# Liz490/multimodal_alzheimer

Measured on AMD Instinct MI355X. Metric: volumes/sec fwd+bwd, 3D-ResNet-10 @128^3 bf16, 1/2/4/8 MI355X; % HBM roofline, higher is better.
Workload: dtype bf16; 1 GPU; BASELINE config 2: Anat_CNN ResNet-10 MRI-only, 1x128^3, batch 8/GPU, weighted CE, Adam, fwd+bwd+step; global_batch=8, parallelism=dp1, step_launch=hip graph replay

## Files before the change

multimodal_alzheimer_amd/csrc/pwgrad.hip:

```cpp
#include "common.h"
#include "patchconv.h"

namespace {

constexpr int PW_KC = 32;
constexpr int PW_TY = 8;
constexpr int PW_XW = 32;
constexpr int PW_YR = PW_TY + 2;
constexpr int PW_XSLOTS = 4;
constexpr int PW_YROW = 128;
constexpr int PW_YST = 2 * PW_XW * PW_YROW;
constexpr int PW_YSLOTS = 4;
constexpr int PW_NTHR = 512;
constexpr uint32_t PW_OOB = 0x80000000u;
template <int MODE>
struct PWC {
  static constexpr bool LAT = MODE == 1, W16 = MODE == 2, W40 = MODE == 3;
  static constexpr int XR = LAT ? 40 : W16 ? 18 : W40 ? 50 : PW_XW + 2;
  static constexpr int SPP = W40 ? 5 : 4;
  static constexpr int YRI = W16 ? 18 : PW_YR;
  static constexpr int XROWS = YRI * XR;
  static constexpr int XDMA = (XROWS + 15) / 16;
  static constexpr int XSLOT = XDMA * 1024;
  static constexpr int Y_OFF = PW_XSLOTS * XSLOT;
  static constexpr int LDS = Y_OFF + PW_YSLOTS * PW_YST;
  static constexpr int NXMAX = (XDMA + 7) / 8;
};

struct PWG {
  int nb, Cs, Nd, D, H, K;
  int zr;
  int ng;
};

__device__ __forceinline__ int pw_wsz128(int r) { return 2 * ((r >> 1) & 1) + 4 * ((r >> 3) & 1); }

template <int MODE>
__global__ __launch_bounds__(PW_NTHR) void pwgrad_kernel(PWG g, const u16* __restrict__ x,
                                                         const u16* __restrict__ dy,
                                                         float* __restrict__ ws) {
  using C = PWC<MODE>;
  constexpr bool LAT = C::LAT, W16 = C::W16, W40 = C::W40;
  constexpr int XR = C::XR, SPP = C::SPP;
  extern __shared__ __attribute__((aligned(16))) char smem[];
  const int tid = threadIdx.x, lane = tid & 63;
  const int wave = __builtin_amdgcn_readfirstlane(tid >> 6);
  const int nci = g.Cs / PW_KC, nco = g.Nd / 64;
  const int nwg = gridDim.x, bid = blockIdx.x;
  const int xcd = bid & 7, qq = nwg >> 3, rr = nwg & 7;
  const int tile = (xcd < rr ? xcd * (qq + 1) : rr * (qq + 1) + (xcd - rr) * qq) + (bid >> 3);
  const int cot = tile % nco, t2 = tile / nco;
  const int cit = t2 % nci, split = t2 / nci;
  const int nyt = LAT ? 2 / g.ng : W16 ? 1 : g.H / PW_TY, nzr = (LAT ? 8 : g.D) / g.zr;
  const int zi = split % nzr, yt = (split / nzr) % nyt, n = split / (nzr * nyt);
  const int rz = LAT ? yt : 0;
  const int co0 = cot * 64, ci0 = cit * PW_KC, y0 = LAT || W16 ? 0 : yt * PW_TY, z0 = zi * g.zr;
  constexpr int VW = LAT || W16 ? 16 : W40 ? 40 : PW_XW;

  const int64_t vox = LAT ? (int64_t)16 * 16 * 16 : (int64_t)g.D * g.H * VW;
  const __amdgpu_buffer_rsrc_t rsx = __builtin_amdgcn_make_buffer_rsrc(
      (void*)(x + n * vox * g.Cs), 0, (int)__builtin_amdgcn_readfirstlane((int)(vox * g.Cs * 2)),
      0x00020000);
  const __amdgpu_buffer_rsrc_t rsy = __builtin_amdgcn_make_buffer_rsrc(
      (void*)(dy + n * vox * g.Nd), 0, (int)__builtin_amdgcn_readfirstlane((int)(vox * g.Nd * 2)),
      0x00020000);
  const uint32_t smem_l = lds_addr_of(smem);

  const int nx = wave + 8 * (C::NXMAX - 1) < C::XDMA ? C::NXMAX : C::NXMAX - 1;
  auto xoff = [&](int h) -> uint32_t {
    const int q = wave + 8 * h, row = 16 * q + (lane >> 2);
    if constexpr (LAT) {
      const int yv = row / XR - 1, ps = row % XR, sg = ps / 10, xv = ps % 10 - 1;
      const bool ok = row < C::XROWS && (unsigned)yv < 8u && (unsigned)xv < 8u;
      const int vy = (sg >> 1) + 2 * yv, vx = (sg & 1) + 2 * xv;
      return ok ? (uint32_t)(((vy * 16 + vx) * g.Cs + ci0 + (lane & 3) * 8) * 2) : PW_OOB;
    } else if constexpr (W16) {
      const int yv = row / XR - 1, xv = row % XR - 1;
      const bool ok = row < C::XROWS && (unsigned)yv < (unsigned)g.H && (unsigned)xv < 16u;
      return ok ? (uint32_t)(((yv * 16 + xv) * g.Cs + ci0 + (lane & 3) * 8) * 2) : PW_OOB;
    } else if constexpr (W40) {
      const int yv = y0 - 1 + row / XR, ps = row % XR, xv = 8 * (ps / 10) + ps % 10 - 1;
      const bool ok = row < C::XROWS && (unsigned)yv < (unsigned)g.H && (unsigned)xv < 40u;
      return ok ? (uint32_t)(((yv * 40 + xv) * g.Cs + ci0 + (lane & 3) * 8) * 2) : PW_OOB;
    } else {
      const int yv = y0 - 1 + row / XR, xv = row % XR - 1;
      const bool ok = row < C::XROWS && (unsigned)yv < (unsigned)g.H &&
                      (unsigned)xv < (unsigned)PW_XW;
      return ok ? (uint32_t)(((yv * PW_XW + xv) * g.Cs + ci0 + (lane & 3) * 8) * 2) : PW_OOB;
    }
  };
  const uint32_t xplane = LAT ? (uint32_t)(16 * 16 * g.Cs * 2) : (uint32_t)(g.H * VW * g.Cs * 2);
  const int gstride = g.zr + 2;
  auto issue_x = [&](int e, int rz) {
    const uint32_t slot = smem_l + (uint32_t)(((unsigned)e % PW_XSLOTS) * C::XSLOT);
    if (LAT && e >= gstride) {
      e -= gstride;
      rz += 1;
    }
    const int zp = z0 - 1 + e;
    const bool zin = !LAT || (unsigned)zp < 8u;
    const uint32_t pz = LAT ? (uint32_t)(rz + 2 * zp) * xplane : (uint32_t)zp * xplane;
#pragma unroll
    for (int h = 0; h < C::NXMAX; ++h)
      if (h < nx)
        buf_lds16_asm(zin ? xoff(h) + pz : PW_OOB, rsx, slot + (uint32_t)((wave + 8 * h) * 1024));
  };
  const int yr = wave * 8 + (lane >> 3);
  const int yvox = LAT ? ((((yr >> 3) & 3) >> 1) + 2 * (yr >> 5)) * 16 + (((yr >> 3) & 3) & 1) +
                             2 * (yr & 7)
                       : yr;
  const uint32_t ylane = (uint32_t)(((W40 ? (lane >> 3) : yvox) * g.Nd + co0 +
                                     ((lane & 7) ^ pw_wsz128(yr)) * 8) * 2);
  auto issue_y = [&](int o, int m, int sl, int rz) {
    uint32_t base;
    if constexpr (W40) {
      const int j = 4 * (2 * m + (wave >> 2)) + (wave & 3);
      base = (uint32_t)((((z0 + o) * g.H + y0 + j / 5) * 40 + 8 * (j % 5)) * g.Nd * 2);
    } else {
      base = LAT ? (uint32_t)(((rz + 2 * (z0 + o)) * 16 + 4 * m) * 16) * (uint32_t)g.Nd * 2
             : W16 ? (uint32_t)(((z0 + o) * g.H + 4 * m) * 16) * (uint32_t)g.Nd * 2
                   : (uint32_t)(((z0 + o) * g.H + y0 + 2 * m) * PW_XW) * (uint32_t)g.Nd * 2;
    }
    buf_lds16_asm(base + ylane, rsy, smem_l + (uint32_t)(C::Y_OFF + sl * PW_YST + wave * 1024));
  };

  const int cf = wave & 1, tg = wave >> 1;
  const int t0 = tg * 7, nt = tg == 3 ? 6 : 7;
  const int lk = lane >> 4, q4 = (lane & 15) >> 2, p4 = lane & 3;
  const int rsel = 8 * lk + q4;
  uint32_t ya_lo[4], ya_hi[4];
#pragma unroll
  for (int i = 0; i < 4; ++i) {
    const int col = i * 16 + 4 * p4;
    ya_lo[i] = (uint32_t)(rsel * PW_YROW + (((col >> 3) ^ pw_wsz128(rsel)) << 4) + (col & 7) * 2);
    ya_hi[i] = (uint32_t)((rsel + 4) * PW_YROW + (((col >> 3) ^ pw_wsz128(rsel + 4)) << 4) +
                          (col & 7) * 2);
  }
  const uint32_t xb = (uint32_t)((LAT ? 10 * lk + q4 : W16 ? 18 * (lk >> 1) + 8 * (lk & 1) + q4
                                  : W40 ? q4 : rsel) *
                                     64 + cf * 32 + 8 * p4);
  uint32_t xk[W40 ? 5 : 1];
#pragma unroll
  for (int kt = 0; kt < (W40 ? 5 : 1); ++kt) {
    const int j = 4 * kt + lk;
    xk[kt] = W40 ? (uint32_t)(((j / 5) * XR + (j % 5) * 10) * 64) : 0u;
  }
  f32x4 acc[4][7];
#pragma unroll
  for (int i = 0; i < 4; ++i)
#pragma unroll
    for (int k = 0; k < 7; ++k) acc[i][k] = f32x4{0.f, 0.f, 0.f, 0.f};

  auto tr8 = [](const char* p) {
    return __builtin_amdgcn_ds_read_tr16_b64_v4bf16((LDS_AS bf16x4*)p);
  };
  auto prologue = [&](int rz) {
    issue_x(0, rz);
    issue_x(1, rz);
    issue_x(2, rz);
    issue_y(0, 0, 0, rz);
    issue_y(0, 1, 1, rz);
  };
  prologue(rz);
  const int ng = LAT ? g.ng : 1;
  const int nstage = ng * g.zr * SPP;

  struct PFr { bf16x8 a[4], b[7]; };
  auto run = [&](auto tgc) {
    constexpr int TG = decltype(tgc)::value;
    constexpr int NT = TG == 3 ? 6 : 7;
    const char* xbase[3];
    auto y_on = [](int t, int yl) constexpr {
      return !LAT || ((unsigned)(yl + (t / 3) % 3 - 1) < 8u);
    };
    auto kread = [&](const char* yimg, auto qc, auto ylc, PFr& f) {
      constexpr int Q = decltype(qc)::value, YL = decltype(ylc)::value;
#pragma unroll
      for (int i = 0; i < 4; ++i)
        f.a[i] = __builtin_shufflevector(tr8(yimg + Q * PW_XW * PW_YROW + ya_lo[i]),
                                         tr8(yimg + Q * PW_XW * PW_YROW + ya_hi[i]), 0, 1, 2, 3,
                                         4, 5, 6, 7);
      auto one = [&](auto kc) {
        constexpr int K = decltype(kc)::value;
        if constexpr (K < NT && y_on(TG * 7 + K, YL)) {
          constexpr int t = TG * 7 + K;
          constexpr int kz = t / 9, ky = (t / 3) % 3, kx = t % 3;
          const char* img;
          if constexpr (W40) {
            constexpr int r0 = ((YL / 5) * 4 + ky) * XR + kx;
            img = xbase[kz] + xk[YL % 5] + r0 * 64;
          } else {
            constexpr int r0 = ((W16 ? 2 : 1) * YL + ky) * XR + kx;
            img = xbase[kz] + r0 * 64;
          }
          f.b[K] = __builtin_shufflevector(tr8(img), tr8(img + 4 * 64), 0, 1, 2, 3, 4, 5, 6, 7);
        }
      };
      one(std::integral_constant<int, 0>{});
      one(std::integral_constant<int, 1>{});
      one(std::integral_constant<int, 2>{});
      one(std::integral_constant<int, 3>{});
      one(std::integral_constant<int, 4>{});
      one(std::integral_constant<int, 5>{});
      one(std::integral_constant<int, 6>{});
    };
    auto kmma = [&](const PFr& f, auto ylc) {
      constexpr int YL = decltype(ylc)::value;
      auto one = [&](auto kc) {
        constexpr int K = decltype(kc)::value;
        if constexpr (K < NT && y_on(TG * 7 + K, YL)) {
#pragma unroll
          for (int i = 0; i < 4; ++i)
            acc[i][K] = __builtin_amdgcn_mfma_f32_16x16x32_bf16(f.a[i], f.b[K], acc[i][K], 0, 0,
                                                                0);
        }
      };
      one(std::integral_constant<int, 0>{});
      one(std::integral_constant<int, 1>{});
      one(std::integral_constant<int, 2>{});
      one(std::integral_constant<int, 3>{});
      one(std::integral_constant<int, 4>{});
      one(std::integral_constant<int, 5>{});
      one(std::integral_constant<int, 6>{});
    };
#pragma unroll 1
    for (int o = 0; o < ng * g.zr; ++o) {
      const bool second = o >= g.zr;
      const int v = o + (second ? 2 : 0);
      if (LAT && o == g.zr) {
        raw_barrier();
        issue_x(v + 1, rz);
        issue_x(v + 2, rz);
      }
#pragma unroll
      for (int j = 0; j < 3; ++j) {
        uint32_t b = (uint32_t)(((unsigned)(v + j) % PW_XSLOTS) * C::XSLOT) + xb;
        asm volatile("v_mov_b32 %0, %1" : "=v"(b) : "v"(b));
        xbase[j] = smem + b;
      }
      const bool xnext = v + 3 < ng * gstride;
      auto stage = [&](auto mc) {
        constexpr int M = decltype(mc)::value;
        const int s = o * SPP + M;
        if (s + 1 >= nstage || (LAT && M == 0 && o == g.zr)) {
          wait_vm_lgkm0<0>();
        } else if ((M == 1 || M == 2) && xnext) {
          if (nx == 4) wait_vm_lgkm0<5>();
          else if (nx == 3) wait_vm_lgkm0<4>();
          else wait_vm_lgkm0<3>();
        } else {
          wait_vm_lgkm0<1>();
        }
        raw_barrier();
        if (s + 2 < nstage) {
          const int p2 = (int)((unsigned)(s + 2) / SPP), g2 = p2 >= g.zr ? 1 : 0;
          issue_y(p2 - g2 * g.zr, (int)((unsigned)(s + 2) % SPP), (int)((unsigned)(s + 2) % PW_YSLOTS), rz + g2);
        }
        if (M == 0 && xnext) issue_x(v + 3, rz);
        int yoff = C::Y_OFF + (int)((unsigned)s % PW_YSLOTS) * PW_YST;
        asm volatile("" : "+s"(yoff));
        const char* yimg = smem + yoff;
        PFr f0, f1;
        kread(yimg, std::integral_constant<int, 0>{}, std::integral_constant<int, 2 * M>{}, f0);
        kread(yimg, std::integral_constant<int, 1>{}, std::integral_constant<int, 2 * M + 1>{},
              f1);
        kmma(f0, std::integral_constant<int, 2 * M>{});
        kmma(f1, std::integral_constant<int, 2 * M + 1>{});
      };
      stage(std::integral_constant<int, 0>{});
      stage(std::integral_constant<int, 1>{});
      stage(std::integral_constant<int, 2>{});
      stage(std::integral_constant<int, 3>{});
      if constexpr (SPP == 5) stage(std::integral_constant<int, 4>{});
    }
  };
  switch (tg) {
    case 0: run(std::integral_constant<int, 0>{}); break;
    case 1: run(std::integral_constant<int, 1>{}); break;
    case 2: run(std::integral_constant<int, 2>{}); break;
    default: run(std::integral_constant<int, 3>{}); break;
  }

  float* out = ws + (int64_t)split * g.Nd * g.K;
  const int lr = lane & 15;
#pragma unroll
  for (int k = 0; k < 7; ++k) {
    if (k < nt) {
      const int kcol = (t0 + k) * g.Cs + ci0 + cf * 16 + lr;
#pragma unroll
      for (int i = 0; i < 4; ++i)
#pragma unroll
        for (int r = 0; r < 4; ++r)
          out[(int64_t)(co0 + i * 16 + lk * 4 + r) * g.K + kcol] = acc[i][k][r];
    }
  }
}

bool pw_on() {
  static const bool v = [] {
    const char* e = getenv("MMAD_PWGRAD");
    return e == nullptr || atoi(e) != 0;
  }();
  return v;
}
bool lat_on() {
  static const bool v = [] {
    const char* e = getenv("MMAD_PWGRAD_LAT");
    return e == nullptr || atoi(e) != 0;
  }();
  return v;
}

bool w16_on() {
  static const bool v = [] {
    const char* e = getenv("MMAD_PWGRAD_W16");
    return e == nullptr || atoi(e) != 0;
  }();
  return v;
}
bool w16_geo(const mmad_patch::Geo& q) {
  return q.KD == 3 && q.KH == 3 && q.KW == 3 && q.dd == 1 && q.dh == 1 && q.dw == 1 &&
         q.pd == 1 && q.ph == 1 && q.pw == 1 && q.Ds == q.Dd && q.Hs == q.Hd && q.Ws == q.Wd &&
         q.Wd == 16 && q.Hd == 16 && q.Dd >= 4;
}
bool w40_on() {
  static const bool v = [] {
    const char* e = getenv("MMAD_PWGRAD_W40");
    return e == nullptr || atoi(e) != 0;
  }();
  return v;
}
bool w40_geo(const mmad_patch::Geo& q) {
  return q.KD == 3 && q.KH == 3 && q.KW == 3 && q.dd == 1 && q.dh == 1 && q.dw == 1 &&
         q.pd == 1 && q.ph == 1 && q.pw == 1 && q.Ds == q.Dd && q.Hs == q.Hd && q.Ws == q.Wd &&
         q.Wd == 40 && q.Hd % PW_TY == 0 && q.Dd >= 4;
}
bool lat_geo(const mmad_patch::Geo& q) {
  return q.KD == 3 && q.KH == 3 && q.KW == 3 && q.dd == 2 && q.dh == 2 && q.dw == 2 &&
         q.pd == 2 && q.ph == 2 && q.pw == 2 && q.Ds == 16 && q.Hs == 16 && q.Ws == 16 &&
         q.Dd == 16 && q.Hd == 16 && q.Wd == 16;
}

int lat_ng(const mmad_patch::Geo& q) {
  static const int force1 = [] {
    const char* e = getenv("MMAD_PWGRAD_LAT_NG");
    return e != nullptr && atoi(e) == 1;
  }();
  if (!lat_geo(q) || force1) return 1;
  return (int64_t)q.nb * (q.Cs / PW_KC) * (q.Nd / 64) >= 256 ? 2 : 1;
}

int pw_zr(const mmad_patch::Geo& q) {
  if (lat_geo(q)) {
    const int64_t base = (int64_t)q.nb * (2 / lat_ng(q)) * (q.Cs / PW_KC) * (q.Nd / 64);
    int zr = 8;
    while (zr > 2 && base * (8 / zr) < 256) zr /= 2;
    return zr;
  }
  const int64_t base =
      (int64_t)q.nb * (w16_geo(q) ? 1 : q.Hd / PW_TY) * (q.Cs / PW_KC) * (q.Nd / 64);
  int zr = q.Dd;
  while (zr > 4 && zr % 2 == 0 && base * (q.Dd / zr) < 256) zr /= 2;
  return zr;
}

}

namespace mmad_pwgrad {

bool ok(const mmad_patch::Geo& q) {
  if (!pw_on()) return false;
  if (q.Cs % PW_KC || q.Nd % 64 || q.Kpad != 27 * q.Cs) return false;
  if (lat_geo(q)) return lat_on() && (int64_t)4096 * std::max(q.Cs, q.Nd) * 2 < (int64_t(1) << 30);
  if (w16_geo(q)) {
    if (!w16_on() || (int64_t)q.Dd * 256 * std::max(q.Cs, q.Nd) * 2 >= (int64_t(1) << 30))
      return false;
    const int zr = pw_zr(q);
    return q.Dd % zr == 0 && zr >= 2;
  }
  if (w40_geo(q)) {
    if (!w40_on() || (int64_t)q.Dd * q.Hd * 40 * std::max(q.Cs, q.Nd) * 2 >= (int64_t(1) << 30))
      return false;
    const int zr = pw_zr(q);
    return q.Dd % zr == 0 && zr >= 2;
  }
  if (q.KD != 3 || q.KH != 3 || q.KW != 3 || q.dd != 1 || q.dh != 1 || q.dw != 1) return false;
  if (q.pd != 1 || q.ph != 1 || q.pw != 1) return false;
  if (q.Ds != q.Dd || q.Hs != q.Hd || q.Ws != q.Wd || q.Wd != PW_XW) return false;
  if (q.Hd % PW_TY || q.Dd < 4) return false;
  if ((int64_t)q.Dd * q.Hd * PW_XW * std::max(q.Cs, q.Nd) * 2 >= (int64_t(1) << 30)) return false;
  const int zr = pw_zr(q);
  return q.Dd % zr == 0 && zr >= 2;
}

int64_t splits(const mmad_patch::Geo& q) {
  if (lat_geo(q)) return (int64_t)q.nb * (2 / lat_ng(q)) * (8 / pw_zr(q));
  if (w16_geo(q)) return (int64_t)q.nb * (q.Dd / pw_zr(q));
  return (int64_t)q.nb * (q.Hd / PW_TY) * (q.Dd / pw_zr(q));
}

int64_t workspace(const mmad_patch::Geo& q) {
  return mmad_pwgrad::splits(q) * q.Nd * 27 * q.Cs * 4;
}

int wgrad(const mmad_patch::Geo& q, const void* x, const void* dy, float* ws, int* nsplit,
          void* stream) {
  if (!mmad_pwgrad::ok(q)) return MMAD_EUNSUPPORTED;
  static const bool attr =
      hipFuncSetAttribute((const void*)pwgrad_kernel<0>,
                          hipFuncAttributeMaxDynamicSharedMemorySize, PWC<0>::LDS) == hipSuccess &&
      hipFuncSetAttribute((const void*)pwgrad_kernel<1>,
                          hipFuncAttributeMaxDynamicSharedMemorySize, PWC<1>::LDS) == hipSuccess &&
      hipFuncSetAttribute((const void*)pwgrad_kernel<2>,
                          hipFuncAttributeMaxDynamicSharedMemorySize, PWC<2>::LDS) == hipSuccess &&
      hipFuncSetAttribute((const void*)pwgrad_kernel<3>,
                          hipFuncAttributeMaxDynamicSharedMemorySize, PWC<3>::LDS) == hipSuccess;
  if (!attr) return MMAD_EUNSUPPORTED;
  const int mode = lat_geo(q) ? 1 : w16_geo(q) ? 2 : w40_geo(q) ? 3 : 0;
  PWG g{};
  g.nb = q.nb; g.Cs = q.Cs; g.Nd = q.Nd; g.D = q.Dd; g.H = q.Hd; g.K = 27 * q.Cs;
  g.zr = pw_zr(q);
  g.ng = lat_ng(q);
  const int64_t sp = mmad_pwgrad::splits(q);
  const int64_t nblk = sp * (q.Cs / PW_KC) * (q.Nd / 64);
  if (mode == 1)
    hipLaunchKernelGGL(pwgrad_kernel<1>, dim3((unsigned)nblk), dim3(PW_NTHR), PWC<1>::LDS,
                       as_stream(stream), g, (const u16*)x, (const u16*)dy, ws);
  else if (mode == 2)
    hipLaunchKernelGGL(pwgrad_kernel<2>, dim3((unsigned)nblk), dim3(PW_NTHR), PWC<2>::LDS,
                       as_stream(stream), g, (const u16*)x, (const u16*)dy, ws);
  else if (mode == 3)
    hipLaunchKernelGGL(pwgrad_kernel<3>, dim3((unsigned)nblk), dim3(PW_NTHR), PWC<3>::LDS,
                       as_stream(stream), g, (const u16*)x, (const u16*)dy, ws);
  else
    hipLaunchKernelGGL(pwgrad_kernel<0>, dim3((unsigned)nblk), dim3(PW_NTHR), PWC<0>::LDS,
                       as_stream(stream), g, (const u16*)x, (const u16*)dy, ws);
  *nsplit = (int)sp;
  return launch_status();
}

}
```

Baseline: 2792 volumes/sec.

## Software-pipeline weight-grad kernel with register double-buffered fragments and larger dy stages

Restructures the pointwise/3D weight-gradient kernel's inner loop so LDS fragment reads for the next k-step are interleaved with MFMAs of the current step, using double-buffered register fragments and sched_group_barrier hints. Dy stages now cover KS (default 4) k-rows per barrier with 3 LDS slots, which halves the number of barriers and waits per plane. Lane-dependent address math is moved into the issue lambdas and the per-i address arrays are replaced by XOR offsets to cut register pressure. Debug macros (PW_NO_READ, PW_NO_MMA, PW_NO_BAR) are added for profiling. In exchange, the larger stage sizes and unrolled pipeline may raise register use or LDS footprint.

```diff
diff --git a/multimodal_alzheimer_amd/csrc/pwgrad.hip b/multimodal_alzheimer_amd/csrc/pwgrad.hip
--- a/multimodal_alzheimer_amd/csrc/pwgrad.hip
+++ b/multimodal_alzheimer_amd/csrc/pwgrad.hip
@@ -9,21 +9,36 @@
 constexpr int PW_YR = PW_TY + 2;
 constexpr int PW_XSLOTS = 4;
 constexpr int PW_YROW = 128;
-constexpr int PW_YST = 2 * PW_XW * PW_YROW;
-constexpr int PW_YSLOTS = 4;
+#ifndef PW_KS0
+#define PW_KS0 4
+#endif
+#ifndef PW_KS1
+#define PW_KS1 4
+#endif
+#ifndef PW_KS2
+#define PW_KS2 4
+#endif
 constexpr int PW_NTHR = 512;
 constexpr uint32_t PW_OOB = 0x80000000u;
 template <int MODE>
 struct PWC {
   static constexpr bool LAT = MODE == 1, W16 = MODE == 2, W40 = MODE == 3;
   static constexpr int XR = LAT ? 40 : W16 ? 18 : W40 ? 50 : PW_XW + 2;
-  static constexpr int SPP = W40 ? 5 : 4;
+  static constexpr int KS = MODE == 0 ? PW_KS0 : MODE == 1 ? PW_KS1 : MODE == 2 ? PW_KS2 : 2;
+  static constexpr int KPP = W40 ? 10 : 8;
+  static constexpr int SPP = KPP / KS;
+  static constexpr int NY = KS / 2;
+  static constexpr int YST = KS * PW_XW * PW_YROW;
+  static constexpr int YSLOTS = KS == 4 ? 3 : 4;
+  static constexpr int PD = YSLOTS - 1;
+  static_assert((KS == 2 || KS == 4) && KPP % KS == 0 && SPP >= PD, "stage length");
   static constexpr int YRI = W16 ? 18 : PW_YR;
   static constexpr int XROWS = YRI * XR;
   static constexpr int XDMA = (XROWS + 15) / 16;
   static constexpr int XSLOT = XDMA * 1024;
   static constexpr int Y_OFF = PW_XSLOTS * XSLOT;
-  static constexpr int LDS = Y_OFF + PW_YSLOTS * PW_YST;
+  static constexpr int LDS = Y_OFF + YSLOTS * YST;
+  static_assert(LDS <= 160 * 1024, "LDS");
   static constexpr int NXMAX = (XDMA + 7) / 8;
 };
 
@@ -34,6 +49,10 @@
 };
 
 __device__ __forceinline__ int pw_wsz128(int r) { return 2 * ((r >> 1) & 1) + 4 * ((r >> 3) & 1); }
+
+__device__ __forceinline__ void pw_consume(const bf16x8& a, const bf16x8& b) {
+  asm volatile("" ::"v"(a), "v"(b));
+}
 
 template <int MODE>
 __global__ __launch_bounds__(PW_NTHR) void pwgrad_kernel(PWG g, const u16* __restrict__ x,
@@ -41,7 +60,8 @@
                                                          float* __restrict__ ws) {
   using C = PWC<MODE>;
   constexpr bool LAT = C::LAT, W16 = C::W16, W40 = C::W40;
-  constexpr int XR = C::XR, SPP = C::SPP;
+  constexpr int XR = C::XR, KS = C::KS, KPP = C::KPP, SPP = C::SPP, NY = C::NY, YST = C::YST;
+  constexpr int YSLOTS = C::YSLOTS, PD = C::PD;
   extern __shared__ __attribute__((aligned(16))) char smem[];
   const int tid = threadIdx.x, lane = tid & 63;
   const int wave = __builtin_amdgcn_readfirstlane(tid >> 6);
@@ -68,6 +88,8 @@
 
   const int nx = wave + 8 * (C::NXMAX - 1) < C::XDMA ? C::NXMAX : C::NXMAX - 1;
   auto xoff = [&](int h) -> uint32_t {
+    int lane = (int)__builtin_amdgcn_mbcnt_hi(~0u, __builtin_amdgcn_mbcnt_lo(~0u, 0u));
+    asm volatile("" : "+v"(lane));
     const int q = wave + 8 * h, row = 16 * q + (lane >> 2);
     if constexpr (LAT) {
       const int yv = row / XR - 1, ps = row % XR, sg = ps / 10, xv = ps % 10 - 1;
@@ -105,13 +127,15 @@
       if (h < nx)
         buf_lds16_asm(zin ? xoff(h) + pz : PW_OOB, rsx, slot + (uint32_t)((wave + 8 * h) * 1024));
   };
-  const int yr = wave * 8 + (lane >> 3);
-  const int yvox = LAT ? ((((yr >> 3) & 3) >> 1) + 2 * (yr >> 5)) * 16 + (((yr >> 3) & 3) & 1) +
-                             2 * (yr & 7)
-                       : yr;
-  const uint32_t ylane = (uint32_t)(((W40 ? (lane >> 3) : yvox) * g.Nd + co0 +
-                                     ((lane & 7) ^ pw_wsz128(yr)) * 8) * 2);
-  auto issue_y = [&](int o, int m, int sl, int rz) {
+  auto issue_y = [&](int o, int m, uint32_t dst, int rz) {
+    int lane = (int)__builtin_amdgcn_mbcnt_hi(~0u, __builtin_amdgcn_mbcnt_lo(~0u, 0u));
+    asm volatile("" : "+v"(lane));
+    const int yr = wave * 8 + (lane >> 3);
+    const int yvox = LAT ? ((((yr >> 3) & 3) >> 1) + 2 * (yr >> 5)) * 16 +
+                               (((yr >> 3) & 3) & 1) + 2 * (yr & 7)
+                         : yr;
+    const uint32_t ylane = (uint32_t)(((W40 ? (lane >> 3) : yvox) * g.Nd + co0 +
+                                       ((lane & 7) ^ pw_wsz128(yr)) * 8) * 2);
     uint32_t base;
     if constexpr (W40) {
       const int j = 4 * (2 * m + (wave >> 2)) + (wave & 3);
@@ -121,30 +145,27 @@
              : W16 ? (uint32_t)(((z0 + o) * g.H + 4 * m) * 16) * (uint32_t)g.Nd * 2
                    : (uint32_t)(((z0 + o) * g.H + y0 + 2 * m) * PW_XW) * (uint32_t)g.Nd * 2;
     }
-    buf_lds16_asm(base + ylane, rsy, smem_l + (uint32_t)(C::Y_OFF + sl * PW_YST + wave * 1024));
+    buf_lds16_asm(base + ylane, rsy, smem_l + (uint32_t)(C::Y_OFF + wave * 1024) + dst);
+  };
+  const int ng = LAT ? g.ng : 1;
+  const int nplanes = ng * g.zr, nstage = nplanes * SPP;
+  auto issue_stage = [&](int sidx, uint32_t dst) {
+    const int p = (int)((unsigned)sidx / SPP), g2 = p >= g.zr ? 1 : 0;
+    const int m0 = (int)((unsigned)sidx % SPP) * NY;
+#pragma unroll
+    for (int h = 0; h < NY; ++h)
+      issue_y(p - g2 * g.zr, m0 + h, dst + (uint32_t)(h * 2 * PW_XW * PW_YROW), rz + g2);
   };
 
   const int cf = wave & 1, tg = wave >> 1;
   const int t0 = tg * 7, nt = tg == 3 ? 6 : 7;
   const int lk = lane >> 4, q4 = (lane & 15) >> 2, p4 = lane & 3;
   const int rsel = 8 * lk + q4;
-  uint32_t ya_lo[4], ya_hi[4];
-#pragma unroll
-  for (int i = 0; i < 4; ++i) {
-    const int col = i * 16 + 4 * p4;
-    ya_lo[i] = (uint32_t)(rsel * PW_YROW + (((col >> 3) ^ pw_wsz128(rsel)) << 4) + (col & 7) * 2);
-    ya_hi[i] = (uint32_t)((rsel + 4) * PW_YROW + (((col >> 3) ^ pw_wsz128(rsel + 4)) << 4) +
-                          (col & 7) * 2);
-  }
-  const uint32_t xb = (uint32_t)((LAT ? 10 * lk + q4 : W16 ? 18 * (lk >> 1) + 8 * (lk & 1) + q4
-                                  : W40 ? q4 : rsel) *
+  const uint32_t ya0 = (uint32_t)(rsel * PW_YROW + ((((4 * p4) >> 3) ^ pw_wsz128(rsel)) << 4) +
+                                  ((4 * p4) & 7) * 2);
+  const uint32_t xb = (uint32_t)((LAT || W40 ? 10 * lk + q4
+                                  : W16 ? 18 * (lk >> 1) + 8 * (lk & 1) + q4 : rsel) *
                                      64 + cf * 32 + 8 * p4);
-  uint32_t xk[W40 ? 5 : 1];
-#pragma unroll
-  for (int kt = 0; kt < (W40 ? 5 : 1); ++kt) {
-    const int j = 4 * kt + lk;
-    xk[kt] = W40 ? (uint32_t)(((j / 5) * XR + (j % 5) * 10) * 64) : 0u;
-  }
   f32x4 acc[4][7];
 #pragma unroll
   for (int i = 0; i < 4; ++i)
@@ -154,124 +175,159 @@
   auto tr8 = [](const char* p) {
     return __builtin_amdgcn_ds_read_tr16_b64_v4bf16((LDS_AS bf16x4*)p);
   };
-  auto prologue = [&](int rz) {
-    issue_x(0, rz);
-    issue_x(1, rz);
-    issue_x(2, rz);
-    issue_y(0, 0, 0, rz);
-    issue_y(0, 1, 1, rz);
-  };
-  prologue(rz);
-  const int ng = LAT ? g.ng : 1;
-  const int nstage = ng * g.zr * SPP;
+  issue_x(0, rz);
+  issue_x(1, rz);
+  issue_x(2, rz);
+#pragma unroll
+  for (int i = 0; i < YSLOTS - 1; ++i)
+    if (i < nstage) issue_stage(i, (uint32_t)(i * YST));
 
   struct PFr { bf16x8 a[4], b[7]; };
   auto run = [&](auto tgc) {
     constexpr int TG = decltype(tgc)::value;
     constexpr int NT = TG == 3 ? 6 : 7;
     const char* xbase[3];
-    auto y_on = [](int t, int yl) constexpr {
-      return !LAT || ((unsigned)(yl + (t / 3) % 3 - 1) < 8u);
-    };
-    auto kread = [&](const char* yimg, auto qc, auto ylc, PFr& f) {
-      constexpr int Q = decltype(qc)::value, YL = decltype(ylc)::value;
-#pragma unroll
-      for (int i = 0; i < 4; ++i)
-        f.a[i] = __builtin_shufflevector(tr8(yimg + Q * PW_XW * PW_YROW + ya_lo[i]),
-                                         tr8(yimg + Q * PW_XW * PW_YROW + ya_hi[i]), 0, 1, 2, 3,
-                                         4, 5, 6, 7);
-      auto one = [&](auto kc) {
-        constexpr int K = decltype(kc)::value;
-        if constexpr (K < NT && y_on(TG * 7 + K, YL)) {
-          constexpr int t = TG * 7 + K;
-          constexpr int kz = t / 9, ky = (t / 3) % 3, kx = t % 3;
-          const char* img;
-          if constexpr (W40) {
-            constexpr int r0 = ((YL / 5) * 4 + ky) * XR + kx;
-            img = xbase[kz] + xk[YL % 5] + r0 * 64;
-          } else {
-            constexpr int r0 = ((W16 ? 2 : 1) * YL + ky) * XR + kx;
-            img = xbase[kz] + r0 * 64;
-          }
-          f.b[K] = __builtin_shufflevector(tr8(img), tr8(img + 4 * 64), 0, 1, 2, 3, 4, 5, 6, 7);
-        }
-      };
-      one(std::integral_constant<int, 0>{});
-      one(std::integral_constant<int, 1>{});
-      one(std::integral_constant<int, 2>{});
-      one(std::integral_constant<int, 3>{});
-      one(std::integral_constant<int, 4>{});
-      one(std::integral_constant<int, 5>{});
-      one(std::integral_constant<int, 6>{});
-    };
-    auto kmma = [&](const PFr& f, auto ylc) {
-      constexpr int YL = decltype(ylc)::value;
-      auto one = [&](auto kc) {
-        constexpr int K = decltype(kc)::value;
-        if constexpr (K < NT && y_on(TG * 7 + K, YL)) {
-#pragma unroll
-          for (int i = 0; i < 4; ++i)
-            acc[i][K] = __builtin_amdgcn_mfma_f32_16x16x32_bf16(f.a[i], f.b[K], acc[i][K], 0, 0,
-                                                                0);
-        }
-      };
-      one(std::integral_constant<int, 0>{});
-      one(std::integral_constant<int, 1>{});
-      one(std::integral_constant<int, 2>{});
-      one(std::integral_constant<int, 3>{});
-      one(std::integral_constant<int, 4>{});
-      one(std::integral_constant<int, 5>{});
-      one(std::integral_constant<int, 6>{});
-    };
-#pragma unroll 1
-    for (int o = 0; o < ng * g.zr; ++o) {
-      const bool second = o >= g.zr;
-      const int v = o + (second ? 2 : 0);
-      if (LAT && o == g.zr) {
-        raw_barrier();
-        issue_x(v + 1, rz);
-        issue_x(v + 2, rz);
-      }
+    auto setx = [&](int v) {
 #pragma unroll
       for (int j = 0; j < 3; ++j) {
         uint32_t b = (uint32_t)(((unsigned)(v + j) % PW_XSLOTS) * C::XSLOT) + xb;
         asm volatile("v_mov_b32 %0, %1" : "=v"(b) : "v"(b));
         xbase[j] = smem + b;
       }
+    };
+    auto y_on = [](int t, int yl) constexpr {
+      return !LAT || ((unsigned)(yl + (t / 3) % 3 - 1) < 8u);
+    };
+    auto ntap = [](int yl) constexpr {
+      int c = 0;
+      for (int k = 0; k < NT; ++k)
+        c += !LAT || ((unsigned)(yl + ((TG * 7 + k) / 3) % 3 - 1) < 8u) ? 1 : 0;
+      return c;
+    };
+    auto aread = [&](const char* yimg, auto qc, auto ic, PFr& f) {
+      constexpr int Q = decltype(qc)::value, I = decltype(ic)::value;
+#ifdef PW_NO_READ
+      asm volatile("" : "=v"(f.a[I]));
+#else
+      uint32_t ya = ya0;
+      asm volatile("" : "+v"(ya));
+      const char* pa = yimg + Q * PW_XW * PW_YROW + (ya ^ (uint32_t)(I << 5));
+      f.a[I] = __builtin_shufflevector(tr8(pa), tr8(pa + 4 * PW_YROW), 0, 1, 2, 3, 4, 5, 6, 7);
+#endif
+    };
+    auto bread = [&](auto ylc, auto kc, PFr& f) {
+      constexpr int YL = decltype(ylc)::value, K = decltype(kc)::value;
+      if constexpr (K < NT && y_on(TG * 7 + K, YL)) {
+#ifdef PW_NO_READ
+        asm volatile("" : "=v"(f.b[K]));
+#else
+        constexpr int t = TG * 7 + K;
+        constexpr int kz = t / 9, ky = (t / 3) % 3, kx = t % 3;
+        const char* img;
+        if constexpr (W40) {
+          constexpr int r0 = ((YL / 5) * 4 + ky) * XR + kx + 40 * (YL % 5);
+          img = xbase[kz] + r0 * 64;
+        } else {
+          constexpr int r0 = ((W16 ? 2 : 1) * YL + ky) * XR + kx;
+          img = xbase[kz] + r0 * 64;
+        }
+        f.b[K] = __builtin_shufflevector(tr8(img), tr8(img + 4 * 64), 0, 1, 2, 3, 4, 5, 6, 7);
+#endif
+      }
+    };
+    auto mma = [&](const PFr& f, auto ylc, auto kc) {
+      constexpr int YL = decltype(ylc)::value, K = decltype(kc)::value;
+      if constexpr (K < NT && y_on(TG * 7 + K, YL)) {
+#ifdef PW_NO_MMA
+#pragma unroll
+        for (int i = 0; i < 4; ++i) pw_consume(f.a[i], f.b[K]);
+#else
+#pragma unroll
+        for (int i = 0; i < 4; ++i)
+          acc[i][K] = __builtin_amdgcn_mfma_f32_16x16x32_bf16(f.a[i], f.b[K], acc[i][K], 0, 0, 0);
+#endif
+      }
+    };
+    auto wait_n = [&](auto bc, bool withx) {
+      constexpr int B = decltype(bc)::value;
+      if (!withx) wait_vm_lgkm0<B>();
+      else if (nx == 4) wait_vm_lgkm0<B + 4>();
+      else if (nx == 3) wait_vm_lgkm0<B + 3>();
+      else wait_vm_lgkm0<B + 2>();
+    };
+    uint32_t ycur = (uint32_t)((YSLOTS - 1) * YST);
+    auto refill = [&](int sn, bool pfirst, int vn) {
+      if (pfirst && vn + 3 < ng * gstride) issue_x(vn + 3, rz);
+      if (sn + PD < nstage) issue_stage(sn + PD, ycur);
+      ycur = ycur + YST == YSLOTS * YST ? 0u : ycur + YST;
+    };
+#ifndef PW_NO_BAR
+    wait_vm_lgkm0<0>();
+    raw_barrier();
+#endif
+    refill(0, true, 0);
+    setx(0);
+    PFr f[2];
+    {
+      uint32_t yoff = C::Y_OFF + ycur;
+      asm volatile("" : "+s"(yoff));
+      [&]<int... K>(std::integer_sequence<int, K...>) {
+        ((K < 4 ? aread(smem + yoff, std::integral_constant<int, 0>{},
+                        std::integral_constant<int, K & 3>{}, f[0]) : (void)0,
+          bread(std::integral_constant<int, 0>{}, std::integral_constant<int, K>{}, f[0])), ...);
+      }(std::make_integer_sequence<int, 7>{});
+    }
+#pragma unroll 1
+    for (int o = 0; o < nplanes; ++o) {
+      const int v = o + (o >= g.zr ? 2 : 0);
+      const int vn = o + 1 + (o + 1 >= g.zr ? 2 : 0);
       const bool xnext = v + 3 < ng * gstride;
-      auto stage = [&](auto mc) {
-        constexpr int M = decltype(mc)::value;
-        const int s = o * SPP + M;
-        if (s + 1 >= nstage || (LAT && M == 0 && o == g.zr)) {
-          wait_vm_lgkm0<0>();
-        } else if ((M == 1 || M == 2) && xnext) {
-          if (nx == 4) wait_vm_lgkm0<5>();
-          else if (nx == 3) wait_vm_lgkm0<4>();
-          else wait_vm_lgkm0<3>();
-        } else {
-          wait_vm_lgkm0<1>();
+      auto kstep = [&](auto ylc) {
+        constexpr int YL = decltype(ylc)::value, M = YL / KS;
+        constexpr bool LASTK = YL % KS == KS - 1, LASTP = YL == KPP - 1;
+        constexpr int YN = LASTP ? 0 : YL + 1;
+        if (LASTK && (!LASTP || o + 1 < nplanes)) {
+          const int s = o * SPP + M;
+#ifndef PW_NO_BAR
+          if (LAT && LASTP && o + 1 == g.zr) {
+            wait_vm_lgkm0<0>();
+            raw_barrier();
+            issue_x(vn + 1, rz);
+            issue_x(vn + 2, rz);
+            wait_vm_lgkm0<0>();
+          } else if (s + PD >= nstage) {
+            wait_vm_lgkm0<0>();
+          } else {
+            wait_n(std::integral_constant<int, (PD - 1) * NY>{}, M <= PD - 2 && xnext);
+          }
+          raw_barrier();
+#endif
+          refill(s + 1, LASTP, vn);
         }
-        raw_barrier();
-        if (s + 2 < nstage) {
-          const int p2 = (int)((unsigned)(s + 2) / SPP), g2 = p2 >= g.zr ? 1 : 0;
-          issue_y(p2 - g2 * g.zr, (int)((unsigned)(s + 2) % SPP), (int)((unsigned)(s + 2) % PW_YSLOTS), rz + g2);
-        }
-        if (M == 0 && xnext) issue_x(v + 3, rz);
-        int yoff = C::Y_OFF + (int)((unsigned)s % PW_YSLOTS) * PW_YST;
+        asm volatile("" ::: "memory");
+        if constexpr (LASTP) setx(vn);
+        uint32_t yoff = C::Y_OFF + ycur;
         asm volatile("" : "+s"(yoff));
         const char* yimg = smem + yoff;
-        PFr f0, f1;
-        kread(yimg, std::integral_constant<int, 0>{}, std::integral_constant<int, 2 * M>{}, f0);
-        kread(yimg, std::integral_constant<int, 1>{}, std::integral_constant<int, 2 * M + 1>{},
-              f1);
-        kmma(f0, std::integral_constant<int, 2 * M>{});
-        kmma(f1, std::integral_constant<int, 2 * M + 1>{});
+        auto tapk = [&](auto kc) {
+          constexpr int K = decltype(kc)::value;
+          constexpr bool ON = K < NT && y_on(TG * 7 + K, YL), ONN = K < NT && y_on(TG * 7 + K, YN);
+          mma(f[YL & 1], std::integral_constant<int, YL>{}, kc);
+          bread(std::integral_constant<int, YN>{}, kc, f[YN & 1]);
+          if constexpr (K < 4)
+            aread(yimg, std::integral_constant<int, YN % KS>{},
+                  std::integral_constant<int, K & 3>{}, f[YN & 1]);
+          if constexpr (ON) __builtin_amdgcn_sched_group_barrier(0x008, 4, 0);
+          if constexpr (ONN || K < 4)
+            __builtin_amdgcn_sched_group_barrier(0x100, (ONN ? 2 : 0) + (K < 4 ? 2 : 0), 0);
+        };
+        [&]<int... K>(std::integer_sequence<int, K...>) {
+          (tapk(std::integral_constant<int, K>{}), ...);
+        }(std::make_integer_sequence<int, 7>{});
       };
-      stage(std::integral_constant<int, 0>{});
-      stage(std::integral_constant<int, 1>{});
-      stage(std::integral_constant<int, 2>{});
-      stage(std::integral_constant<int, 3>{});
-      if constexpr (SPP == 5) stage(std::integral_constant<int, 4>{});
+      [&]<int... Y>(std::integer_sequence<int, Y...>) {
+        (kstep(std::integral_constant<int, Y>{}), ...);
+      }(std::make_integer_sequence<int, KPP>{});
     }
   };
   switch (tg) {
```

After: 2797 volumes/sec (median of 6 runs). About the same (+0.2%).
